# chechaohp/gan-ode

Measured on AMD Instinct MI355X. Metric: generated videos/sec (16-frame clips), higher is better.
Workload: dtype f32

## Files before the change

### gan-ode_amd/_lib.py

```python
from __future__ import annotations

import ctypes as C
import os
import sys

_HERE = os.path.dirname(os.path.abspath(__file__))
LIB_PATH = os.path.join(_HERE, "lib", "libgode.so")

i32, i64, f32, ptr = C.c_int32, C.c_int64, C.c_float, C.c_void_p
cint, u32, u64 = C.c_int, C.c_uint32, C.c_uint64

ACT_NONE, ACT_RELU, ACT_LRELU, ACT_TANH_OUT = 0, 1, 2, 3
ACT_TANH, ACT_SIGMOID = 4, 5
ACT_LRELU01 = 6
EPI_RAW, EPI_TANH = 0, 1
FPROP, DGRAD = 0, 1
PACK_BORDER = 0x100
OP_IGEMM, OP_WGRAD, OP_BN_FINALIZE, OP_BN_BWD, OP_ODE_FWD, OP_ODE_BWD, OP_BCE, OP_ADAM, OP_PACK = range(1, 10)
OP_ODERNN_FWD, OP_ODERNN_BWD, OP_BN_APPLY, OP_COL2IM = 10, 11, 12, 13
OP_SDE_FWD, OP_SDE_BWD = 14, 15
OP_CDE_FWD, OP_CDE_BWD = 16, 17
OP_WGAN = 18
OP_GRU_FWD, OP_GRU_BWD = 19, 20
OP_DNOISE = 21
OP_CATEG, OP_CE = 22, 23
OP_CHSTATS, OP_CBN_EMBED, OP_CBN_EMBED_BWD, OP_CBN_APPLY, OP_CBN_BWD, OP_GRES_OUT, OP_GRES_OUT_BWD, OP_SN_FWD, OP_SN_BWD = range(24, 33)
OP_FC_ACT, OP_FC_ACT_BWD, OP_BCE_PROB = 33, 34, 35
OP_BCE_T = 36
OP_RESIZE_U8, OP_CLIP_GATHER = 37, 38
RESIZE_MAX_TAPS = 32
REC_ADAM_NOISE = -1
ODE_NPARAM = 2672
ODERNN_NPARAM = 2176
SDE_NPARAM = 3216
CDE_NPARAM = 7536
CDE_MAX_N = 4096
GRU_NPARAM = 1632
SN_BWD_BLOCKS = 64
ODE_METHODS = {"rk4": 0, "dopri5": 1, "euler": 2, "midpoint": 3}
ODE_RHS = {"mlp": 0, "tanh": 1}
ODE_RHS_TANH_NPARAM = 2400


def ode_method_code(name):
# ... 27 lines not shown
    KIND, FN = OP_IGEMM, "gode_igemm"


class WgradOp(_Op):
    _fields_ = [("g", ConvGeom), ("act", i32), ("xform_on_y", i32), ("splits", i32), ("accumulate", i32),
                ("x", ptr), ("y", ptr), ("scale", ptr), ("shift", ptr), ("work", ptr), ("dw", ptr),
                ("co_perm", ptr), ("co_canon", i64), ("xs", i64 * 5)]
    KIND, FN = OP_WGRAD, "gode_wgrad"


class BnFinalizeOp(_Op):
    _fields_ = [("stats", ptr), ("rows", i32), ("ncols", i32), ("C", i32), ("count", i64), ("gamma", ptr),
                ("beta", ptr), ("running_mean", ptr), ("running_var", ptr), ("num_batches_tracked", ptr),
                ("mean", ptr), ("invstd", ptr), ("scale", ptr), ("shift", ptr), ("momentum", f32), ("eps", f32),
                ("training", i32), ("pad_", i32), ("groups", i32), ("rows0", i32), ("nseg", i32), ("order", i32),
                ("count1", i64), ("seg", i32 * 24), ("stats1", ptr), ("rows1", i32), ("pad3_", i32)]
    KIND, FN = OP_BN_FINALIZE, "gode_bn_finalize"


class BnBwdOp(_Op):
    _fields_ = [("g", ptr), ("y", ptr), ("M", i64), ("C", i32), ("act", i32), ("gamma", ptr), ("mean", ptr),
                ("invstd", ptr), ("scale", ptr), ("shift", ptr), ("dgamma", ptr), ("dbeta", ptr), ("work", ptr),
                ("accumulate", i32), ("eval_mode", i32), ("gin", ptr), ("groups", i32), ("pad2_", i32), ("M0", i64),
                ("r1_s", ptr), ("r1_w", ptr), ("r1_H", i32), ("r1_W", i32), ("r1_h", i32), ("r1_wd", i32), ("r1_off", i32),
                ("pad3_", i32)]
    KIND, FN = OP_BN_BWD, "gode_bn_bwd"


class OdeParams(C.Structure):
    _fields_ = [(n, ptr) for n in "Wa ba Wb bb W1 b1 W2 b2".split()]


# ... 271 lines not shown
    "gode_scale": ([ptr, ptr, i64, f32, cint, ptr], cint),
    "gode_adam_multi": ([ptr, i32, i64, f32, f32, f32, f32, f32, f32, i32, ptr], cint),
    "gode_adam_multi_dev": ([ptr, i32, i64, f32, f32, f32, f32, f32, ptr, ptr], cint),
    "gode_adam_noise_multi": ([ptr, i32, i64, f32, f32, f32, f32, f32, f32, i32, u64, u32, u32, f32, ptr], cint),
    "gode_adam_noise_multi_dev": ([ptr, i32, i64, f32, f32, f32, f32, f32, ptr, u64, u32, f32, ptr], cint),
    "gode_param_noise": ([ptr, i64, u64, u32, u32, i64, f32, i32, ptr], cint),
    "gode_dnoise_normals": ([ptr, i64, u64, u32, u32, u32, i64, i32, ptr], cint),
    "gode_ode_step_chunks": ([ptr, i64], i64),
    "gode_ode_step": ([ptr, i32, i64, i32, f32, f32, f32, f32, f32, ptr, ptr], cint),
    "gode_axpy_multi": ([ptr, i32, i64, f32, ptr, ptr, f32, ptr, ptr, ptr], cint),
    "gode_run": ([ptr, ptr, i32, ptr], cint),
    "gode_lanes_create": ([ptr], cint),
    "gode_lanes_destroy": ([ptr], cint),
    "gode_lanes_stream": ([ptr], ptr),
    "gode_run_lanes": ([ptr, ptr, ptr, i32, i32, i32, i32, ptr], cint),
    "gode_version": (None, cint),
    "gode_sizeof": ([cint], cint),
}

EXPORTS = [st.FN for st in _OPS] + list(_PROTOS)

_lib = None


def lib():
    global _lib
    if _lib is not None:
        return _lib
    if not os.path.exists(LIB_PATH):
        raise RuntimeError(f"{LIB_PATH} is missing: build it with `python __graft_entry__.py` "
# ... 63 lines not shown

class Lanes:

    _free = {}

    def __init__(self, device_index):
        self.device_index = device_index
        pool = Lanes._free.setdefault(device_index, [])
        if pool:
            self.handle = pool.pop()
        else:
            self.handle = ptr()
            check(lib().gode_lanes_create(C.byref(self.handle)), "gode_lanes_create")
        self.stream_ptr = lib().gode_lanes_stream(self.handle)

    def __del__(self):
        h, self.handle = getattr(self, "handle", None), None
        if h and not sys.is_finalizing():
            Lanes._free.setdefault(self.device_index, []).append(h)


class LanesProgram(Program):

    def __init__(self, ops, n_front, release_after):
        super().__init__(ops)
        self.n_front, self.release_after = int(n_front), int(release_after)

    def run_lanes(self, lanes, mode, stream):
        global LAUNCHES
        LAUNCHES += 1
        check(lib().gode_run_lanes(lanes.handle, self.kinds, self.ptrs, self.n, self.n_front, self.release_after, mode,
                                   stream), "gode_run_lanes")


def run_one(op, stream):
    global LAUNCHES
    LAUNCHES += 1
    if op.KIND == OP_PACK:
        launch = lambda: check(lib().gode_pack_weights(C.byref(op.g), op.dir, op.w, op.wpack, op.co_perm, op.co_canon,
                                                       stream), "gode_pack_weights")
        return _traced(op, stream, launch) if TRACE is not None else launch()
    if TRACE is not None:
        return _traced(op, stream, lambda: _run_one(op, stream))
    _run_one(op, stream)


def _run_one(op, stream):
# ... 2 lines not shown
```

### gan-ode_amd/csrc/api.hip

```cpp
#include "common.h"

extern "C" int gode_version(void) { return GODE_VERSION; }

extern "C" int gode_sizeof(int kind) {
  switch (kind) {
    case 0: return (int)sizeof(gode_conv_geom);
    case -1: return (int)sizeof(gode_adam_noise_tensor);
    case GODE_OP_PACK: return (int)sizeof(gode_pack_op);
#define GODE_SIZEOF_ROW_(name, value, op_t, fn) case GODE_OP_##name: return (int)sizeof(op_t);
    GODE_OPS(GODE_SIZEOF_ROW_)
#undef GODE_SIZEOF_ROW_
  }
  return GODE_E_KIND;
}

extern "C" int gode_pack_batch_(const gode_pack_op* const* ops, int n, void* stream);

static int run_range(const int32_t* kinds, const void* const* ops, int lo, int hi, void* stream) {
  for (int i = lo; i < hi; ++i) {
    int rc;
    switch (kinds[i]) {
#define GODE_RUN_ROW_(name, value, op_t, fn) case GODE_OP_##name: rc = fn((const op_t*)ops[i], stream); break;
      GODE_OPS(GODE_RUN_ROW_)
#undef GODE_RUN_ROW_
// ... 8 lines not shown
    }
    if (rc != 0) return rc > 0 ? rc : rc * 1000 - i;
  }
  return 0;
}

extern "C" int gode_run(const int32_t* kinds, const void* const* ops, int32_t n, void* stream) {
  if (n < 0 || (n > 0 && (!kinds || !ops))) return GODE_E_ARG;
  return run_range(kinds, ops, 0, n, stream);
}

struct gode_lanes {
  hipStream_t side;
  hipEvent_t ev_entry, ev_front, ev_release;
  bool released;
};

#define GODE_HIP_TRY(expr)                          \
  do {                                              \
    hipError_t e__ = (expr);                        \
    if (e__ != hipSuccess) return (int)e__;         \
  } while (0)

extern "C" int gode_lanes_destroy(gode_lanes* l) {
  if (!l) return GODE_E_ARG;
  int rc = 0;
  if (l->side) {
    hipError_t e = hipStreamSynchronize(l->side);
    if (e != hipSuccess) rc = (int)e;
  }
// ... 23 lines not shown
}

extern "C" void* gode_lanes_stream(gode_lanes* l) { return l ? (void*)l->side : nullptr; }

extern "C" int gode_run_lanes(gode_lanes* l, const int32_t* kinds, const void* const* ops, int32_t n, int32_t n_front,
                              int32_t release_after, int32_t mode, void* stream) {
  if (!l || n < 0 || (n > 0 && (!kinds || !ops)) || n_front < 0 || n_front > n || release_after < n_front ||
      release_after >= n || (mode != GODE_LANES_ORDERED && mode != GODE_LANES_OVERLAP))
    return GODE_E_ARG;
  hipStream_t main = (hipStream_t)stream;
  hipStreamCaptureStatus cap = hipStreamCaptureStatusNone;
  if (hipStreamIsCapturing(main, &cap) != hipSuccess) {
    (void)hipGetLastError();
    cap = hipStreamCaptureStatusActive;
  }
  if (cap != hipStreamCaptureStatusNone) {
    l->released = false;
    return run_range(kinds, ops, 0, n, stream);
  }
  const bool overlap = mode == GODE_LANES_OVERLAP && l->released;
  l->released = false;
  if (overlap) {
    GODE_HIP_TRY(hipStreamWaitEvent(l->side, l->ev_release, 0));
  } else {
    GODE_HIP_TRY(hipEventRecord(l->ev_entry, main));
    GODE_HIP_TRY(hipStreamWaitEvent(l->side, l->ev_entry, 0));
  }
  int rc = run_range(kinds, ops, 0, n_front, (void*)l->side);
  if (rc != 0) return rc;
  GODE_HIP_TRY(hipEventRecord(l->ev_front, l->side));
  GODE_HIP_TRY(hipStreamWaitEvent(main, l->ev_front, 0));
  rc = run_range(kinds, ops, n_front, release_after + 1, stream);
  if (rc != 0) return rc;
  GODE_HIP_TRY(hipEventRecord(l->ev_release, main));
  l->released = true;
  rc = run_range(kinds, ops, release_after + 1, n, stream);
  if (rc != 0) l->released = false;
  return rc;
}
```

### gan-ode_amd/csrc/elementwise.hip

```cpp
#include "common.h"
#include "philox.h"
#include "col2im_plan.h"

__global__ void __launch_bounds__(256) bn_finalize_kernel(const gode_bn_finalize_op a) {
  const int c = blockIdx.x, tid = threadIdx.x;
  __shared__ double red[2][256];
  if (a.training) {
    const int reps = a.ncols / a.C;
    const int ngroups = a.groups == 2 ? 2 : 1;
    for (int gi = 0; gi < ngroups; ++gi) {
      const int grp = ngroups == 2 ? (a.order ? 1 - gi : gi) : 0;
      double s1 = 0.0, s2 = 0.0;
      const int nseg = (ngroups == 2 && !a.stats1) ? (a.nseg > 0 ? a.nseg : 1) : 1;
      for (int sg = 0; sg < nseg; ++sg) {
        int r_lo, r_hi;
        if (ngroups == 1 || a.stats1) { r_lo = 0; r_hi = (grp == 1 && a.stats1) ? a.rows1 : a.rows; }
        else if (a.nseg > 0) { r_lo = grp == 0 ? a.seg[3 * sg] : a.seg[3 * sg + 1]; r_hi = grp == 0 ? a.seg[3 * sg + 1] : a.seg[3 * sg + 2]; }
        else { r_lo = grp == 0 ? 0 : a.rows0; r_hi = grp == 0 ? a.rows0 : a.rows; }
        const float* st = (grp == 1 && a.stats1) ? a.stats1 : a.stats;
        const int stride = (grp == 1 && a.stats1) ? a.rows1 : a.rows;
        const int nr = r_hi - r_lo;
        const int64_t items = (int64_t)nr * reps;
        for (int64_t i = tid; i < items; i += 256) {
          const int rep = (int)(i / nr); const int r = r_lo + (int)(i - (int64_t)rep * nr);
// ... 8 lines not shown
      for (int s = 128; s > 0; s >>= 1) {
        if (tid < s) { red[0][tid] += red[0][tid + s]; red[1][tid] += red[1][tid + s]; }
        __syncthreads();
      }
      if (tid == 0) {
        const double n = (double)((grp == 1 && a.count1 > 0) ? a.count1 : a.count);
        const double mean = red[0][0] / n;
        double var = red[1][0] / n - mean * mean;
        if (var < 0.0) var = 0.0;
        const float invstd = (float)(1.0 / sqrt(var + (double)a.eps));
        const float g = a.gamma ? a.gamma[c] : 1.f, b = a.beta ? a.beta[c] : 0.f;
        const float sc = g * invstd;
        const int o = grp * a.C + c;
        a.mean[o] = (float)mean; a.invstd[o] = invstd;
        a.scale[o] = sc; a.shift[o] = b - (float)mean * sc;
        if (a.running_mean) {
          const double unbiased = n > 1.0 ? var * n / (n - 1.0) : var;
          a.running_mean[c] = (1.f - a.momentum) * a.running_mean[c] + a.momentum * (float)mean;
          a.running_var[c] = (1.f - a.momentum) * a.running_var[c] + a.momentum * (float)unbiased;
        }
        if (c == 0 && a.num_batches_tracked) *a.num_batches_tracked += 1;
      }
    }
  } else if (tid == 0) {
    const float invstd = 1.f / sqrtf(a.running_var[c] + a.eps);
    const float g = a.gamma ? a.gamma[c] : 1.f, b = a.beta ? a.beta[c] : 0.f;
    const float sc = g * invstd;
    const int ngroups = a.groups == 2 ? 2 : 1;
    for (int grp = 0; grp < ngroups; ++grp) {
      const int o = grp * a.C + c;
      if (a.mean) a.mean[o] = a.running_mean[c];
      if (a.invstd) a.invstd[o] = invstd;
      a.scale[o] = sc; a.shift[o] = b - a.running_mean[c] * sc;
    }
  }
}

extern "C" int gode_bn_finalize(const gode_bn_finalize_op* op, void* stream) {
  if (!op || op->C <= 0 || !op->scale || !op->shift) return GODE_E_ARG;
  if (op->training) {
    if (!op->stats || !op->mean || !op->invstd || op->ncols % op->C != 0 || op->count <= 0) return GODE_E_ARG;
    if (op->stats1 && (op->groups != 2 || op->rows1 <= 0 || op->rows <= 0)) return GODE_E_ARG;
    if (op->groups == 2 && !op->stats1 && op->nseg == 0 && (op->rows0 <= 0 || op->rows0 >= op->rows)) return GODE_E_ARG;
    if (op->groups == 2 && (op->nseg < 0 || op->nseg > 8)) return GODE_E_ARG;
    for (int i = 0; op->groups == 2 && i < op->nseg; ++i)
      if (!(0 <= op->seg[3 * i] && op->seg[3 * i] <= op->seg[3 * i + 1] && op->seg[3 * i + 1] <= op->seg[3 * i + 2] && op->seg[3 * i + 2] <= op->rows)) return GODE_E_ARG;
  } else if (!op->running_mean || !op->running_var) return GODE_E_ARG;
  hipLaunchKernelGGL(bn_finalize_kernel, dim3(op->C), dim3(256), 0, (hipStream_t)stream, *op);
  GODE_LAUNCH_CHECK();
  return 0;
}

__global__ void __launch_bounds__(256) bn_apply_kernel(const gode_bn_apply_op a) {
  const int64_t n4 = a.M * a.C / 4;
  const float neg = gode_act_neg_slope(a.act);
  for (int64_t i = (int64_t)blockIdx.x * 256 + threadIdx.x; i < n4; i += (int64_t)gridDim.x * 256) {
    const int c = (int)((i * 4) % a.C) + ((a.M0 > 0 && i * 4 >= a.M0 * a.C) ? a.C : 0);
    f32x4 v = *reinterpret_cast<const f32x4*>(a.y + i * 4);
    f32x4 sc = {1.f, 1.f, 1.f, 1.f}, sh = {0.f, 0.f, 0.f, 0.f};
    if (a.scale) { sc = *reinterpret_cast<const f32x4*>(a.scale + c); sh = *reinterpret_cast<const f32x4*>(a.shift + c); }
#pragma unroll
    for (int e = 0; e < 4; ++e) { const float t = v[e] * sc[e] + sh[e]; v[e] = fmaxf(t, t * neg); }
    *reinterpret_cast<f32x4*>(a.out + i * 4) = v;
// ... 619 lines not shown
```

### gan-ode_amd/engine.py

```python
from __future__ import annotations

import ctypes as C
import os
from dataclasses import dataclass
from typing import List, Optional, Sequence

import numpy as np
import torch

from . import _lib as L

BORDER_TAKE_DEAD_TAPS = 0.06
BORDER_TAKE_TILES_PER_SLOT = 2.0


def border_value(g) -> int:
    lib = L.lib()
    if lib.gode_igemm_dead_taps(C.byref(L.IgemmOp(g=g, dir=L.DGRAD, tile=0))) < BORDER_TAKE_DEAD_TAPS:
        return 1
    info = (C.c_int32 * 4)()
    L.check(lib.gode_igemm_launch_info(C.byref(L.IgemmOp(g=g, dir=L.DGRAD, tile=0, border=2)), info))
    return 2 if info[0] and info[2] >= BORDER_TAKE_TILES_PER_SLOT * info[3] else 1


# ... 62 lines not shown
    return (i - back) % n


def lane_gate(prev_lanes, prev_copy_pending, before_prev_copy_pending):
    return bool(prev_copy_pending) if prev_lanes else bool(before_prev_copy_pending)


def lane_mode(*, enabled, trace, recording, categorical, grad, keep, fixed_grid_ode, splittable, prev_lanes, launches_between,
              repacked, versions_same, same_stream, gpu_behind=True):
    if (not enabled or trace or recording or categorical or grad or keep or not fixed_grid_ode or not splittable
            or not gpu_behind):
        return LANE_SINGLE
    if prev_lanes and launches_between == 0 and not repacked and versions_same and same_stream:
        return LANE_OVERLAP
    return LANE_ORDERED


@dataclass
class LayerSpec:
    geom: L.ConvGeom
    fwd_dir: int
    act: int
    has_bn: bool
    epilogue: int = L.EPI_RAW
    co_perm: Optional[torch.Tensor] = None
    noise: bool = False

    def out_dims(self):
        g = self.geom
        if self.fwd_dir == L.FPROP:
# ... 134 lines not shown
            L.Program(stale).run(st)
        return bool(stale)

    def front_split(self, prog, pre_ops):
        first = prog.ops[0] if prog.ops else None
        if (self.split or self.groups != 1 or self.noisy or self.x_in is None or len(prog.ops) < 2
                or not isinstance(first, L.IgemmOp) or first.out != dptr(self.y[0])):
            return None
        lib = L.lib()
        ops = list(pre_ops) + list(prog.ops)
        n_front = len(pre_ops) + 1
        written = front_writes(ops[:n_front], uses_work=lambda op: lib.gode_igemm_work_size(C.byref(op)) > 0)
        extents = {t.data_ptr(): t.numel() * t.element_size()
                   for t in (self.x_in, self.y[0], self.stats[0], self._ig_work) if t is not None}
        return ops, n_front, release_after(ops, n_front, written, extents)

    @staticmethod
    def _ncols(s: LayerSpec):
        g = s.geom
        if s.fwd_dir == L.FPROP:
            return g.Co
        fullk = (g.Do == 1 and g.Ho == 1 and g.Wo == 1 and g.pd == 0 and g.ph == 0 and g.pw == 0 and
                 g.Di == g.kd and g.Hi == g.kh and g.Wi == g.kw and g.kd * g.kh * g.kw > 1)
        return g.kd * g.kh * g.kw * g.Ci if fullk else g.Ci

    def _materialize(self, l):
        if l + 1 >= len(self.specs):
            return False
        if self.specs[l + 1].noise:
            return True
# ... 266 lines not shown
            if k is not None:
                x, xs = inputs[k]
                op.x = x.data_ptr()
                for i in range(5):
                    op.xs[i] = int(xs[i])

    def forward(self, training: bool, x: Optional[torch.Tensor] = None, x_strides=None, pre_ops_program=None,
                x2: Optional[torch.Tensor] = None, x2_strides=None, noise=None):
        prog, out, _ = self.begin_forward(training, x, x_strides, x2, x2_strides, noise)
        st = stream_ptr()
        if pre_ops_program is not None:
            pre_ops_program.run(st)
        prog.run(st)
        return self.end_forward(out, training)

    def begin_forward(self, training: bool, x=None, x_strides=None, x2=None, x2_strides=None, noise=None):
        self._refresh()
        if training not in self._fwd:
            self._fwd[training] = self._build_fwd(training)
        prog, patch = self._fwd[training]
        if self.noisy:
            if noise is None:
                raise RuntimeError("this plan applies instance noise: forward() needs its noise arguments")
            self._patch_noise(patch, noise, [(x, x_strides), (x2, x2_strides)])
        out = torch.empty(self.out_dims, dtype=torch.float32, device=self.device)
        patch["last"].out = out.data_ptr()
        if "last2" in patch:
            patch["last2"][0].out = out.data_ptr() + patch["last2"][1]
        if self.x_in is None and self.x0n is None:
            first = patch["first"]
            first.src = x.data_ptr()
            for i in range(5):
                first.gs[i] = int(x_strides[i])
        if self.x_in is None:
            self._x_user, self._x_strides = x.detach(), tuple(int(v) for v in x_strides)
            if self.groups == 2:
                if self.x0n is None:
                    second = patch["first2"]
                    second.src = x2.data_ptr()
                    for i in range(5):
# ... 267 lines not shown
```

### gan-ode_amd/modules.py

```python
from __future__ import annotations

import contextlib
import ctypes as C
import math
import os
from typing import Optional

import numpy as np
import torch
import torch.nn as nn

from . import _lib as L
from .engine import (LANE_ORDERED, LANE_OVERLAP, LANE_SINGLE, ConvStack, LayerParams, LayerSpec, conv_out, dptr, lane_gate,
                     lane_mode, make_geom, ring_back, stream_ptr)

Z_COLS = 96
Z_CATEG0 = 66
MAX_CATEG = Z_COLS - Z_CATEG0
ODE_METHODS = L.ODE_METHODS
_SAMPLE_LANES_ENV = os.environ.get("GODE_SAMPLE_LANES", "1") != "0"


def ode_method_code(name):
    return L.ode_method_code(name)


def _require_gpu(t: torch.Tensor, what: str):
    if not t.is_cuda:
        raise RuntimeError(f"{what}: this implementation runs only on an MI355X through libgode.so; move the module "
                           "to the GPU with .cuda() (there is no CPU or PyTorch fallback)")


class _Pool:

    MAX_PLANS = 6
# ... 170 lines not shown
_ODE_GRAD_OFFS = [(0, 1024, (64, 16)), (1024, 64, (64,)), (1088, 1024, (16, 64)), (2112, 16, (16,)),
                  (2128, 256, (16, 16)), (2384, 16, (16,)), (2400, 256, (16, 16)), (2656, 16, (16,))]
_PRENET_NPARAM = 2128


class _GenPlan:

    zcols = 68
    rows_in_traj = True
    rhs = property(lambda self: L.ode_rhs_code("tanh" if _is_one_layer(self.gen.ode_fn) else "mlp"))
    nparam = property(lambda self: L.ODE_RHS_TANH_NPARAM if self.rhs else L.ODE_NPARAM)
    grad_offs = property(lambda self: _ODE_GRAD_OFFS[:6] if self.rhs else _ODE_GRAD_OFFS)
    grads_from_first_present = False
    multi, multi_always = ("ode", L.OdeFwdOp, L.OdeBwdOp), False

    def __init__(self, gen: "VideoGenerator", n_traj: int, T: int, select: bool, zbuf=None, x=None):
        dev = gen.main[0].weight.device
        self.gen, self.n, self.T, self.select, self.device = gen, n_traj, T, select, dev
        self.rows = n_traj if select else n_traj * T
        f32 = dict(dtype=torch.float32, device=dev)
        self.ncat = int(getattr(gen, "dim_z_category", 0)) if x is None else 0
        self.labels = None
        self.x, self.content, self.sel, self.cls = x, None, None, None
        self._ring = []
        if x is None:
            xs = self._x_shape(n_traj, T)
            sx, sc, ss, sk = _input_slices(int(np.prod(xs)), n_traj)
            nin = sk.stop if self.ncat else sk.start
            self._in = torch.zeros(nin, **f32)
            self.x, self.content = self._in[sx].view(xs), self._in[sc].view(n_traj, 50)
            self.sel = self._in[ss].view(torch.int32) if select else None
# ... 2 lines not shown
        self._ring_i = 0
        self.stack = None
        if x is not None:
            self._zbuf, self._zcols = torch.empty(n_traj * T, self.zcols, **f32), self.zcols
        elif zbuf is not None:
            self._zbuf, self._zcols = zbuf, Z_COLS
        else:
            self.stack = ConvStack(gen._decoder_specs(self.rows), gen._decoder_params(), dev, owns_input=True,
                                   pack_cache=gen._pool.pack_cache, two_lane_backward=True)
            self._zbuf, self._zcols = self.stack.x_in, Z_COLS
        self._alloc()
        self._ode_ptrs = None
        self.busy = False
        self._lanes = self._side = self._lane_prog = self._lane_prev = None
        self.lane_calls = {LANE_OVERLAP: 0, LANE_ORDERED: 0, LANE_SINGLE: 0}
        self._lanes_ok = type(self) is _GenPlan and self.stack is not None and not self.ncat and _SAMPLE_LANES_ENV
        self.lanes_made_late = False
        if self._lanes_ok and gen.sample_lanes:
            self._make_lanes()

    @staticmethod
    def _x_shape(n_traj, T):
        return (n_traj, 16)

    def _alloc(self):
        f32 = dict(dtype=torch.float32, device=self.device)
        self.traj = torch.empty(self.n, self.T, 16, **f32)
        tt = torch.linspace(0, 1, self.T).float()
        self.dt = (tt[1:] - tt[:-1]).to(self.device) if self.T > 1 else torch.zeros(1, **f32)
        self.ode_work = torch.empty(L.lib().gode_ode_bwd_work_size(self.n), **f32)

    def _params(self):
        g = self.gen
# ... 88 lines not shown
        if feed is not None and feed.recording:
            nfl = self._in.numel()
            pin, dev = feed.noise_region(self.gen, self.select, self.n, self.T, nfl)
            _pack_inputs(pin, x_host, content_host, sel_host, cls_host)
            self._in.copy_(dev)
        else:
            slot = self._ring[self._ring_i]
            self._ring_i = (self._ring_i + 1) % len(self._ring)
            if slot["ev"] is not None:
                slot["ev"].synchronize()
            _pack_inputs(slot["buf"], x_host, content_host, sel_host, cls_host)
            self._in.copy_(slot["buf"], non_blocking=True)
            if slot["ev"] is None:
                slot["ev"] = torch.cuda.Event()
            slot["ev"].record()

    def forward(self, x_host, content_host, sel_host, training, keep, cls_host=None, no_grad=False):
        if x_host is None:
            torch.cuda.current_stream().wait_event(self._latent_ev)
            out = self.stack.forward(training)
            self._lane_prev = None
        elif self._lanes_possible(keep, no_grad):
            out = self._forward_lanes(x_host, content_host, sel_host, training)
        else:
            self.stage_inputs(x_host, content_host, sel_host, cls_host)
            out = self.stack.forward(training, pre_ops_program=self.fwd_prog)
            self._lane_prev = None
            self.lane_calls[LANE_SINGLE] += 1
        self.busy = keep
        return out

    def _lanes_possible(self, keep, no_grad):
        gen = self.gen
        if (not no_grad or keep or not gen.sample_lanes or gen._one_stream or not self._lanes_ok or L.TRACE is not None
                or gen.ode_method == "dopri5"):
            return False
        if gen.sample_lanes != "always" and not lane_gate(self._lane_prev is not None, self._copy_pending(1),
                                                          self._copy_pending(2)):
            return False
        feed = getattr(gen, "_feed", None)
        if (feed is not None and feed.recording) or torch.cuda.is_current_stream_capturing():
            return False
        if self._lanes is None:
            self._make_lanes()
            self.lanes_made_late = True
        return True

    def _copy_pending(self, back):
        ev = self._ring[ring_back(self._ring_i, len(self._ring), back)]["ev"]
        return ev is not None and not ev.query()

    def _make_lanes(self):
        with torch.cuda.device(self.device):
            self._lanes = L.Lanes(torch.cuda.current_device())
        self._side = torch.cuda.ExternalStream(self._lanes.stream_ptr, device=self.device)

    def _front_versions(self):
        ts = [t for t in self._params() if t is not None] + [self.stack.params[0].weight]
        return tuple((t._version, getattr(t, "_gode_ver", 0), t.data_ptr()) for t in ts)

    def _forward_lanes(self, x_host, content_host, sel_host, training):
        self._programs()
        prev, self._lane_prev = self._lane_prev, None
        between = L.LAUNCHES - prev["mark"] if prev is not None else -1
        prog, out, repacked = self.stack.begin_forward(training)
        st = stream_ptr()
        cache = self._lane_prog
        if cache is None or cache[0] is not prog or cache[1] is not self.fwd_prog:
            split = self.stack.front_split(prog, self.fwd_prog.ops)
# ... 19 lines not shown
        return self.stack.end_forward(out, training)

    def _stage_on_side(self, ordered, x_host, content_host, sel_host):
        slot = self._ring[self._ring_i]
        self._ring_i = (self._ring_i + 1) % len(self._ring)
        if slot["ev"] is not None:
            slot["ev"].synchronize()
        _pack_inputs(slot["buf"], x_host, content_host, sel_host)
        if ordered:
            self._side.wait_stream(torch.cuda.current_stream())
        with torch.cuda.stream(self._side):
            self._in.copy_(slot["buf"], non_blocking=True)
            if slot["ev"] is None:
                slot["ev"] = torch.cuda.Event()
            slot["ev"].record()

    def _decoder_pass_done(self):
        cb = getattr(self.gen, "_on_decoder_grads", None)
        if cb is not None:
            self.gen._decoder_passes_left -= 1
            if self.gen._decoder_passes_left == 0:
                cb()

    def backward(self, gout, arena=None):
        if arena is not None:
            into = _grads_into(arena, self.gen._decoder_params())
            _, _, gz = self.stack.backward(gout, need_input_grad=True, into=into)
            self._decoder_pass_done()
            self.latent_backward(gz.data_ptr(), arena, gz)
            self.busy = False
# ... 277 lines not shown
        if not isinstance(self.linear, nn.Identity):
            ode += [self.linear[0].weight, self.linear[0].bias, self.linear[2].weight, self.linear[2].bias]
        ode += _ode_fn_tensors(self.ode_fn)
        return self._decoder_list(), ode

    def _apply(self, fn, *a, **k):
        r = super()._apply(fn, *a, **k)
        if hasattr(self, "_pool"):
            self._pool.clear()
            self.__dict__.pop("_labels", None)
            self.__dict__.pop("_latent_plans", None)
            self.__dict__.pop("_prefetched", None)
        return r

    def lane_stats(self):
        out = {LANE_OVERLAP: 0, LANE_ORDERED: 0, LANE_SINGLE: 0, "lanes_objects": 0, "lanes_objects_made_late": 0}
        for plans in self._pool.plans.values():
            for p in plans:
                for k, v in getattr(p, "lane_calls", {}).items():
                    out[k] += v
                out["lanes_objects"] += getattr(p, "_lanes", None) is not None
                out["lanes_objects_made_late"] += bool(getattr(p, "lanes_made_late", False))
        return out

    @contextlib.contextmanager
    def one_stream(self):
        self._one_stream += 1
        try:
            yield
        finally:
            self._one_stream -= 1

    def invalidate_packs(self):
        for k in [k for k in self._pool.pack_cache if k[0] == "ver"]:
            del self._pool.pack_cache[k]
        for plans in self._pool.plans.values():
            for p in plans:
                if getattr(p, "_lane_prev", None) is not None:
                    p._lane_prev = None

    def _zero_labels(self, n, device):
        key = (n, device)
        t = self.__dict__.setdefault("_labels", {}).get(key)
        if t is None:
            t = self._labels[key] = torch.zeros(n, dtype=torch.float64, device=device)
        return t

    _gode_direct_grads = True

    def _arena_tail(self):
        return self._param_list()[1]

    def _draw(self, num_samples, video_len):
        content = np.random.normal(0, 1, (num_samples, self.dim_z_content)).astype(np.float32)
# ... 1025 lines not shown
```

### include/gode.h

```cpp
#ifndef GODE_H
#define GODE_H
#include <stdint.h>
#ifdef __cplusplus
extern "C" {
#endif

#define GODE_VERSION 105

enum { GODE_OK = 0, GODE_E_ARG = -1, GODE_E_SHAPE = -2, GODE_E_KIND = -3 };
enum { GODE_ACT_NONE = 0, GODE_ACT_RELU = 1, GODE_ACT_LRELU = 2,
       GODE_ACT_TANH_OUT = 3 ,
       GODE_ACT_TANH = 4, GODE_ACT_SIGMOID = 5 ,
       GODE_ACT_LRELU01 = 6  };
enum { GODE_EPI_RAW = 0, GODE_EPI_TANH = 1 };
enum { GODE_FPROP = 0, GODE_DGRAD = 1 };
enum { GODE_PACK_BORDER = 0x100 };

typedef struct gode_conv_geom {
  int32_t N, Ci, Co;
  int32_t Di, Hi, Wi;
  int32_t Do, Ho, Wo;
  int32_t kd, kh, kw;
  int32_t sd, sh, sw;
  int32_t pd, ph, pw;
// ... 40 lines not shown
  int64_t xs[5];
} gode_wgrad_op;
int gode_wgrad(const gode_wgrad_op* op, void* stream);
int64_t gode_wgrad_work_size(const gode_wgrad_op* op);
int gode_wgrad_auto_splits(const gode_conv_geom* g);

typedef struct gode_bn_finalize_op {
  const float* stats; int32_t rows, ncols, C; int64_t count;
  const float* gamma; const float* beta;
  float* running_mean; float* running_var; int64_t* num_batches_tracked;
  float* mean; float* invstd; float* scale; float* shift;
  float momentum, eps; int32_t training, pad_;
  int32_t groups, rows0;
  int32_t nseg, order; int64_t count1; int32_t seg[24];
  const float* stats1; int32_t rows1, pad3_;
} gode_bn_finalize_op;
int gode_bn_finalize(const gode_bn_finalize_op* op, void* stream);

typedef struct gode_bn_apply_op {
  const float* y; float* out; const float* scale; const float* shift; int64_t M; int32_t C, act;
  int64_t M0;
} gode_bn_apply_op;
int gode_bn_apply(const gode_bn_apply_op* op, void* stream);

typedef struct gode_col2im_op {
  const float* cols; float* out;
  int32_t N, Hi, Wi, Ho, Wo, C, kh, kw, sh, sw, ph, pw;
  int32_t epilogue, pad_;
  int32_t Di, Do, kd, sd, pd, pad2_;
} gode_col2im_op;
int gode_col2im(const gode_col2im_op* op, void* stream);
int gode_col2im_launch_kind(const gode_col2im_op* op, int32_t* kind);
// ... 323 lines not shown
  X(CE,            23, gode_ce_op,            gode_ce_logits)     \
  X(CHSTATS,       24, gode_chstats_op,       gode_chstats)       \
  X(CBN_EMBED,     25, gode_cbn_embed_op,     gode_cbn_embed)     \
  X(CBN_EMBED_BWD, 26, gode_cbn_embed_bwd_op, gode_cbn_embed_bwd) \
  X(CBN_APPLY,     27, gode_cbn_apply_op,     gode_cbn_apply)     \
  X(CBN_BWD,       28, gode_cbn_bwd_op,       gode_cbn_bwd)       \
  X(GRES_OUT,      29, gode_gres_out_op,      gode_gres_out)      \
  X(GRES_OUT_BWD,  30, gode_gres_out_bwd_op,  gode_gres_out_bwd)  \
  X(SN_FWD,        31, gode_sn_op,            gode_sn_fwd)        \
  X(SN_BWD,        32, gode_sn_bwd_op,        gode_sn_bwd)        \
  X(FC_ACT,        33, gode_fc_act_op,        gode_fc_act)        \
  X(FC_ACT_BWD,    34, gode_fc_act_bwd_op,    gode_fc_act_bwd)    \
  X(BCE_PROB,      35, gode_bce_prob_op,      gode_bce_prob)      \
  X(BCE_T,         36, gode_bce_t_op,         gode_bce_logits_t)  \
  X(RESIZE_U8,     37, gode_resize_u8_op,     gode_resize_u8)     \
  X(CLIP_GATHER,   38, gode_clip_gather_op,   gode_clip_gather)
#define GODE_ENUM_ROW_(name, value, op_t, fn) GODE_OP_##name = value,
enum { GODE_OPS(GODE_ENUM_ROW_) GODE_OP_PACK = 9 };
#undef GODE_ENUM_ROW_
typedef struct gode_pack_op {
  gode_conv_geom g; int32_t dir , co_canon; const float* w; float* wpack; const int32_t* co_perm;
} gode_pack_op;
int gode_run(const int32_t* kinds, const void* const* ops, int32_t n, void* stream);

typedef struct gode_lanes gode_lanes;
enum { GODE_LANES_ORDERED = 0, GODE_LANES_OVERLAP = 1 };
int gode_lanes_create(gode_lanes** out);
int gode_lanes_destroy(gode_lanes* lanes);
void* gode_lanes_stream(gode_lanes* lanes);
int gode_run_lanes(gode_lanes* lanes, const int32_t* kinds, const void* const* ops, int32_t n, int32_t n_front,
                   int32_t release_after, int32_t mode, void* stream);

int gode_version(void);
int gode_sizeof(int kind);

#ifdef __cplusplus
}
#endif
#endif
```

Before: 39280.

## Double-buffer generator sampling across two plans with deferred BN running-stat update

Adds a paired execution mode in which consecutive training-mode sampling calls alternate between two plan copies on separate side streams. When overlap is allowed, each call's front waits on the peer's entry event rather than its own, so two forward passes can run concurrently. BN finalize now writes the batch variance to a scratch buffer, and a single trailing BN_RUNNING kernel on the main stream applies the running-mean/var updates in order, keeping the shared running statistics race-free. This costs a second set of buffers and lanes, one extra launch per call, and more complex ordering logic.

```diff
diff --git a/gan-ode_amd/_lib.py b/gan-ode_amd/_lib.py
--- a/gan-ode_amd/_lib.py
+++ b/gan-ode_amd/_lib.py
@@ -28,6 +28,8 @@
 OP_FC_ACT, OP_FC_ACT_BWD, OP_BCE_PROB = 33, 34, 35
 OP_BCE_T = 36
 OP_RESIZE_U8, OP_CLIP_GATHER = 37, 38
+OP_BN_RUNNING = 39
+BN_RUNNING_MAX = 8
 RESIZE_MAX_TAPS = 32
 REC_ADAM_NOISE = -1
 ODE_NPARAM = 2672
@@ -85,8 +87,18 @@
                 ("beta", ptr), ("running_mean", ptr), ("running_var", ptr), ("num_batches_tracked", ptr),
                 ("mean", ptr), ("invstd", ptr), ("scale", ptr), ("shift", ptr), ("momentum", f32), ("eps", f32),
                 ("training", i32), ("pad_", i32), ("groups", i32), ("rows0", i32), ("nseg", i32), ("order", i32),
-                ("count1", i64), ("seg", i32 * 24), ("stats1", ptr), ("rows1", i32), ("pad3_", i32)]
+                ("count1", i64), ("seg", i32 * 24), ("stats1", ptr), ("rows1", i32), ("pad3_", i32), ("batch_var", ptr)]
     KIND, FN = OP_BN_FINALIZE, "gode_bn_finalize"
+
+
+class BnRunningLayer(C.Structure):
+    _fields_ = [("mean", ptr), ("var", ptr), ("running_mean", ptr), ("running_var", ptr), ("num_batches_tracked", ptr),
+                ("C", i32), ("pad_", i32)]
+
+
+class BnRunningOp(_Op):
+    _fields_ = [("layer", BnRunningLayer * BN_RUNNING_MAX), ("n", i32), ("momentum", f32)]
+    KIND, FN = OP_BN_RUNNING, "gode_bn_running"
 
 
 class BnBwdOp(_Op):
@@ -388,6 +400,7 @@
     "gode_lanes_destroy": ([ptr], cint),
     "gode_lanes_stream": ([ptr], ptr),
     "gode_run_lanes": ([ptr, ptr, ptr, i32, i32, i32, i32, ptr], cint),
+    "gode_run_pair": ([ptr, ptr, ptr, ptr, i32, i32, i32, ptr], cint),
     "gode_version": (None, cint),
     "gode_sizeof": ([cint], cint),
 }
@@ -481,6 +494,15 @@
             check(lib().gode_lanes_create(C.byref(self.handle)), "gode_lanes_create")
         self.stream_ptr = lib().gode_lanes_stream(self.handle)
 
+    _shared = {}
+
+    @classmethod
+    def shared(cls, device_index, second):
+        key = (device_index, bool(second))
+        if key not in cls._shared:
+            cls._shared[key] = cls(device_index)
+        return cls._shared[key]
+
     def __del__(self):
         h, self.handle = getattr(self, "handle", None), None
         if h and not sys.is_finalizing():
@@ -498,6 +520,19 @@
         LAUNCHES += 1
         check(lib().gode_run_lanes(lanes.handle, self.kinds, self.ptrs, self.n, self.n_front, self.release_after, mode,
                                    stream), "gode_run_lanes")
+
+
+class PairProgram(Program):
+
+    def __init__(self, ops, n_tail=1):
+        super().__init__(ops)
+        self.n_tail = int(n_tail)
+
+    def run_pair(self, lanes, peer, mode, stream):
+        global LAUNCHES
+        LAUNCHES += 1
+        check(lib().gode_run_pair(lanes.handle, None if peer is None else peer.handle, self.kinds, self.ptrs, self.n,
+                                  self.n_tail, mode, stream), "gode_run_pair")
 
 
 def run_one(op, stream):
diff --git a/gan-ode_amd/csrc/api.hip b/gan-ode_amd/csrc/api.hip
--- a/gan-ode_amd/csrc/api.hip
+++ b/gan-ode_amd/csrc/api.hip
@@ -46,6 +46,7 @@
   hipStream_t side;
   hipEvent_t ev_entry, ev_front, ev_release;
   bool released;
+  bool entered;
 };
 
 #define GODE_HIP_TRY(expr)                          \
@@ -99,6 +100,7 @@
     (void)hipGetLastError();
     cap = hipStreamCaptureStatusActive;
   }
+  l->entered = false;
   if (cap != hipStreamCaptureStatusNone) {
     l->released = false;
     return run_range(kinds, ops, 0, n, stream);
@@ -123,3 +125,30 @@
   if (rc != 0) l->released = false;
   return rc;
 }
+
+extern "C" int gode_run_pair(gode_lanes* l, gode_lanes* peer, const int32_t* kinds, const void* const* ops, int32_t n,
+                             int32_t n_tail, int32_t mode, void* stream) {
+  if (!l || peer == l || n < 2 || !kinds || !ops || n_tail < 1 || n_tail >= n ||
+      (mode != GODE_LANES_ORDERED && mode != GODE_LANES_OVERLAP))
+    return GODE_E_ARG;
+  hipStream_t main = (hipStream_t)stream;
+  hipStreamCaptureStatus cap = hipStreamCaptureStatusNone;
+  if (hipStreamIsCapturing(main, &cap) != hipSuccess) {
+    (void)hipGetLastError();
+    cap = hipStreamCaptureStatusActive;
+  }
+  l->released = false;
+  l->entered = false;
+  if (cap != hipStreamCaptureStatusNone) return run_range(kinds, ops, 0, n, stream);
+  const bool overlap = mode == GODE_LANES_OVERLAP && peer && peer->entered;
+  GODE_HIP_TRY(hipEventRecord(l->ev_entry, main));
+  GODE_HIP_TRY(hipStreamWaitEvent(l->side, overlap ? peer->ev_entry : l->ev_entry, 0));
+  int rc = run_range(kinds, ops, 0, n - n_tail, (void*)l->side);
+  GODE_HIP_TRY(hipEventRecord(l->ev_front, l->side));
+  GODE_HIP_TRY(hipStreamWaitEvent(main, l->ev_front, 0));
+  if (rc != 0) return rc;
+  rc = run_range(kinds, ops, n - n_tail, n, stream);
+  if (rc != 0) return rc;
+  l->entered = true;
+  return 0;
+}
diff --git a/gan-ode_amd/csrc/elementwise.hip b/gan-ode_amd/csrc/elementwise.hip
--- a/gan-ode_amd/csrc/elementwise.hip
+++ b/gan-ode_amd/csrc/elementwise.hip
@@ -1,6 +1,18 @@
 #include "common.h"
 #include "philox.h"
 #include "col2im_plan.h"
+
+__device__ __forceinline__ float bn_running_mean_update(float run, float momentum, float batch_mean) {
+#pragma clang fp contract(off)
+  const float keep = (1.f - momentum) * run;
+  const float add = momentum * batch_mean;
+  return add + keep;
+}
+__device__ __forceinline__ float bn_running_var_update(float run, float momentum, float unbiased) {
+#pragma clang fp contract(off)
+  const float keep = (1.f - momentum) * run;
+  return __builtin_fmaf(momentum, unbiased, keep);
+}
 
 __global__ void __launch_bounds__(256) bn_finalize_kernel(const gode_bn_finalize_op a) {
   const int c = blockIdx.x, tid = threadIdx.x;
@@ -46,12 +58,16 @@
         const int o = grp * a.C + c;
         a.mean[o] = (float)mean; a.invstd[o] = invstd;
         a.scale[o] = sc; a.shift[o] = b - (float)mean * sc;
-        if (a.running_mean) {
-          const double unbiased = n > 1.0 ? var * n / (n - 1.0) : var;
-          a.running_mean[c] = (1.f - a.momentum) * a.running_mean[c] + a.momentum * (float)mean;
-          a.running_var[c] = (1.f - a.momentum) * a.running_var[c] + a.momentum * (float)unbiased;
+        if (a.batch_var) {
+          a.batch_var[c] = (float)(n > 1.0 ? var * n / (n - 1.0) : var);
+        } else {
+          if (a.running_mean) {
+            const double unbiased = n > 1.0 ? var * n / (n - 1.0) : var;
+            a.running_mean[c] = bn_running_mean_update(a.running_mean[c], a.momentum, (float)mean);
+            a.running_var[c] = bn_running_var_update(a.running_var[c], a.momentum, (float)unbiased);
+          }
+          if (c == 0 && a.num_batches_tracked) *a.num_batches_tracked += 1;
         }
-        if (c == 0 && a.num_batches_tracked) *a.num_batches_tracked += 1;
       }
     }
   } else if (tid == 0) {
@@ -78,7 +94,32 @@
     for (int i = 0; op->groups == 2 && i < op->nseg; ++i)
       if (!(0 <= op->seg[3 * i] && op->seg[3 * i] <= op->seg[3 * i + 1] && op->seg[3 * i + 1] <= op->seg[3 * i + 2] && op->seg[3 * i + 2] <= op->rows)) return GODE_E_ARG;
   } else if (!op->running_mean || !op->running_var) return GODE_E_ARG;
+  if (op->batch_var && (!op->training || op->groups == 2 || op->nseg != 0 || op->stats1)) return GODE_E_ARG;
   hipLaunchKernelGGL(bn_finalize_kernel, dim3(op->C), dim3(256), 0, (hipStream_t)stream, *op);
+  GODE_LAUNCH_CHECK();
+  return 0;
+}
+
+__global__ void __launch_bounds__(256) bn_running_kernel(const gode_bn_running_op a) {
+  for (int l = 0; l < a.n; ++l) {
+    const gode_bn_running_layer& y = a.layer[l];
+    if (y.running_mean)
+      for (int c = threadIdx.x; c < y.C; c += 256) {
+        y.running_mean[c] = bn_running_mean_update(y.running_mean[c], a.momentum, y.mean[c]);
+        y.running_var[c] = bn_running_var_update(y.running_var[c], a.momentum, y.var[c]);
+      }
+    if (threadIdx.x == 0 && y.num_batches_tracked) *y.num_batches_tracked += 1;
+    __syncthreads();
+  }
+}
+
+extern "C" int gode_bn_running(const gode_bn_running_op* op, void* stream) {
+  if (!op || op->n <= 0 || op->n > GODE_BN_RUNNING_MAX) return GODE_E_ARG;
+  for (int l = 0; l < op->n; ++l) {
+    const gode_bn_running_layer& y = op->layer[l];
+    if (y.C <= 0 || (y.running_mean && (!y.running_var || !y.mean || !y.var))) return GODE_E_ARG;
+  }
+  hipLaunchKernelGGL(bn_running_kernel, dim3(1), dim3(256), 0, (hipStream_t)stream, *op);
   GODE_LAUNCH_CHECK();
   return 0;
 }
diff --git a/gan-ode_amd/engine.py b/gan-ode_amd/engine.py
--- a/gan-ode_amd/engine.py
+++ b/gan-ode_amd/engine.py
@@ -100,6 +100,25 @@
     if prev_lanes and launches_between == 0 and not repacked and versions_same and same_stream:
         return LANE_OVERLAP
     return LANE_ORDERED
+
+
+def pair_turn(prev_turn):
+    return 0 if prev_turn is None else 1 - prev_turn
+
+
+def pair_wait(turn, overlap):
+    return 1 - turn if overlap else turn
+
+
+def pair_schedule(calls):
+    out, entry, prev = [], {}, None
+    for m, (fresh, may_overlap) in enumerate(calls):
+        turn = pair_turn(None if fresh else prev)
+        overlap = bool(may_overlap) and not fresh and (1 - turn) in entry
+        entry[turn] = m
+        out.append((turn, entry[pair_wait(turn, overlap)]))
+        prev = turn
+    return out
 
 
 @dataclass
@@ -264,6 +283,31 @@
         extents = {t.data_ptr(): t.numel() * t.element_size()
                    for t in (self.x_in, self.y[0], self.stats[0], self._ig_work) if t is not None}
         return ops, n_front, release_after(ops, n_front, written, extents)
+
+    def pair_program(self, prog, pre_ops):
+        if self.split or self.groups != 1 or self.noisy or self.x_in is None or len(prog.ops) < 2:
+            return None
+        fins = [op for op in prog.ops if isinstance(op, L.BnFinalizeOp)]
+        if not fins or len(fins) > L.BN_RUNNING_MAX or any(not f.training or f.groups == 2 or f.nseg or f.stats1 for f in fins):
+            return None
+        if getattr(self, "_bvar", None) is None:
+            self._bvar = {}
+        run = L.BnRunningOp(n=len(fins), momentum=self.momentum)
+        ops, k = list(pre_ops), -1
+        for op in prog.ops:
+            if isinstance(op, L.BnFinalizeOp):
+                k += 1
+                slot = self._bvar.get(k)
+                if slot is None or slot.numel() != op.C:
+                    slot = self._bvar[k] = torch.empty(op.C, dtype=torch.float32, device=self.device)
+                d = L.BnFinalizeOp.from_buffer_copy(op)
+                d.batch_var = slot.data_ptr()
+                y = run.layer[k]
+                y.mean, y.var, y.C = op.mean, slot.data_ptr(), op.C
+                y.running_mean, y.running_var, y.num_batches_tracked = op.running_mean, op.running_var, op.num_batches_tracked
+                op = d
+            ops.append(op)
+        return ops + [run]
 
     @staticmethod
     def _ncols(s: LayerSpec):
@@ -560,7 +604,7 @@
         prog.run(st)
         return self.end_forward(out, training)
 
-    def begin_forward(self, training: bool, x=None, x_strides=None, x2=None, x2_strides=None, noise=None):
+    def begin_forward(self, training: bool, x=None, x_strides=None, x2=None, x2_strides=None, noise=None, out_stream=None):
         self._refresh()
         if training not in self._fwd:
             self._fwd[training] = self._build_fwd(training)
@@ -569,7 +613,13 @@
             if noise is None:
                 raise RuntimeError("this plan applies instance noise: forward() needs its noise arguments")
             self._patch_noise(patch, noise, [(x, x_strides), (x2, x2_strides)])
-        out = torch.empty(self.out_dims, dtype=torch.float32, device=self.device)
+        if out_stream is None:
+            out = torch.empty(self.out_dims, dtype=torch.float32, device=self.device)
+        else:
+            cur = torch.cuda.current_stream()
+            with torch.cuda.stream(out_stream):
+                out = torch.empty(self.out_dims, dtype=torch.float32, device=self.device)
+            out.record_stream(cur)
         patch["last"].out = out.data_ptr()
         if "last2" in patch:
             patch["last2"][0].out = out.data_ptr() + patch["last2"][1]
diff --git a/gan-ode_amd/modules.py b/gan-ode_amd/modules.py
--- a/gan-ode_amd/modules.py
+++ b/gan-ode_amd/modules.py
@@ -12,13 +12,14 @@
 
 from . import _lib as L
 from .engine import (LANE_ORDERED, LANE_OVERLAP, LANE_SINGLE, ConvStack, LayerParams, LayerSpec, conv_out, dptr, lane_gate,
-                     lane_mode, make_geom, ring_back, stream_ptr)
+                     lane_mode, make_geom, pair_turn, stream_ptr)
 
 Z_COLS = 96
 Z_CATEG0 = 66
 MAX_CATEG = Z_COLS - Z_CATEG0
 ODE_METHODS = L.ODE_METHODS
 _SAMPLE_LANES_ENV = os.environ.get("GODE_SAMPLE_LANES", "1") != "0"
+_PAIR_DEFAULT = True
 
 
 def ode_method_code(name):
@@ -219,7 +220,7 @@
     grads_from_first_present = False
     multi, multi_always = ("ode", L.OdeFwdOp, L.OdeBwdOp), False
 
-    def __init__(self, gen: "VideoGenerator", n_traj: int, T: int, select: bool, zbuf=None, x=None):
+    def __init__(self, gen: "VideoGenerator", n_traj: int, T: int, select: bool, zbuf=None, x=None, lanes=None):
         dev = gen.main[0].weight.device
         self.gen, self.n, self.T, self.select, self.device = gen, n_traj, T, select, dev
         self.rows = n_traj if select else n_traj * T
@@ -252,9 +253,17 @@
         self.busy = False
         self._lanes = self._side = self._lane_prog = self._lane_prev = None
         self.lane_calls = {LANE_OVERLAP: 0, LANE_ORDERED: 0, LANE_SINGLE: 0}
+        self._peer = self._pair_prog = self._pair_prev = None
+        self._pair_refused = False
+        self._owner = self
+        self.pair_calls = {LANE_OVERLAP: 0, LANE_ORDERED: 0}
+        self._copies = []
         self._lanes_ok = type(self) is _GenPlan and self.stack is not None and not self.ncat and _SAMPLE_LANES_ENV
         self.lanes_made_late = False
-        if self._lanes_ok and gen.sample_lanes:
+        self._peer_lanes = None
+        if lanes is not None:
+            self._make_lanes(lanes)
+        elif self._lanes_ok and gen.sample_lanes:
             self._make_lanes()
 
     @staticmethod
@@ -373,18 +382,29 @@
             if slot["ev"] is None:
                 slot["ev"] = torch.cuda.Event()
             slot["ev"].record()
+            self._note_copy(slot["ev"])
+
+    def _note_copy(self, ev):
+        own = self._owner
+        own._copies = own._copies[-1:] + [ev]
 
     def forward(self, x_host, content_host, sel_host, training, keep, cls_host=None, no_grad=False):
         if x_host is None:
             torch.cuda.current_stream().wait_event(self._latent_ev)
             out = self.stack.forward(training)
-            self._lane_prev = None
+            self._lane_prev = self._pair_prev = None
         elif self._lanes_possible(keep, no_grad):
-            out = self._forward_lanes(x_host, content_host, sel_host, training)
+            knob = self.gen.sample_lanes
+            if (knob == "pair" or (_PAIR_DEFAULT and knob != "always")) and self._pair_possible(training):
+                self._lane_prev = None
+                out = self._forward_pair(x_host, content_host, sel_host, training)
+            else:
+                self._pair_prev = None
+                out = self._forward_lanes(x_host, content_host, sel_host, training)
         else:
             self.stage_inputs(x_host, content_host, sel_host, cls_host)
             out = self.stack.forward(training, pre_ops_program=self.fwd_prog)
-            self._lane_prev = None
+            self._lane_prev = self._pair_prev = None
             self.lane_calls[LANE_SINGLE] += 1
         self.busy = keep
         return out
@@ -394,8 +414,8 @@
         if (not no_grad or keep or not gen.sample_lanes or gen._one_stream or not self._lanes_ok or L.TRACE is not None
                 or gen.ode_method == "dopri5"):
             return False
-        if gen.sample_lanes != "always" and not lane_gate(self._lane_prev is not None, self._copy_pending(1),
-                                                          self._copy_pending(2)):
+        if gen.sample_lanes not in ("always", "pair") and not lane_gate(
+                self._lane_prev is not None or self._pair_prev is not None, self._copy_pending(1), self._copy_pending(2)):
             return False
         feed = getattr(gen, "_feed", None)
         if (feed is not None and feed.recording) or torch.cuda.is_current_stream_capturing():
@@ -406,12 +426,15 @@
         return True
 
     def _copy_pending(self, back):
-        ev = self._ring[ring_back(self._ring_i, len(self._ring), back)]["ev"]
+        ev = self._copies[-back] if len(self._copies) >= back else None
         return ev is not None and not ev.query()
 
-    def _make_lanes(self):
+    def _make_lanes(self, lanes=None):
         with torch.cuda.device(self.device):
-            self._lanes = L.Lanes(torch.cuda.current_device())
+            self._lanes = lanes if lanes is not None else L.Lanes.shared(torch.cuda.current_device(), False)
+            knob = self.gen.sample_lanes
+            if lanes is None and (knob == "pair" or (_PAIR_DEFAULT and knob != "always")):
+                self._peer_lanes = L.Lanes.shared(torch.cuda.current_device(), True)
         self._side = torch.cuda.ExternalStream(self._lanes.stream_ptr, device=self.device)
 
     def _front_versions(self):
@@ -461,6 +484,51 @@
             if slot["ev"] is None:
                 slot["ev"] = torch.cuda.Event()
             slot["ev"].record()
+        self._note_copy(slot["ev"])
+
+    def _pair_possible(self, training):
+        return training and not self._pair_refused and self.stack._G2 is False and not self.stack.noisy
+
+    def _pair_versions(self):
+        ts = [t for t in self._params() if t is not None]
+        for p in self.stack.params:
+            ts += [t for t in (p.weight, p.gamma, p.beta) if t is not None]
+        return tuple((t._version, getattr(t, "_gode_ver", 0), t.data_ptr()) for t in ts)
+
+    def _forward_pair(self, x_host, content_host, sel_host, training):
+        prev, self._pair_prev = self._pair_prev, None
+        turn = pair_turn(None if prev is None else prev["turn"])
+        if turn == 1 and self._peer is None:
+            if self._peer_lanes is None:
+                with torch.cuda.device(self.device):
+                    self._peer_lanes = L.Lanes.shared(torch.cuda.current_device(), True)
+            peer = self._peer = type(self)(self.gen, self.n, self.T, self.select, lanes=self._peer_lanes)
+            peer._owner = self
+        plan = self._peer if turn else self
+        plan._programs()
+        between = L.LAUNCHES - prev["mark"] if prev is not None else -1
+        prog, out, repacked = plan.stack.begin_forward(training, out_stream=plan._side)
+        st = stream_ptr()
+        cache = plan._pair_prog
+        if cache is None or cache[0] is not prog or cache[1] is not plan.fwd_prog:
+            ops = plan.stack.pair_program(prog, plan.fwd_prog.ops)
+            if ops is None:
+                self._pair_refused = True
+                return self._forward_lanes(x_host, content_host, sel_host, training)
+            cache = plan._pair_prog = (prog, plan.fwd_prog, L.PairProgram(ops, 1))
+            prev = None
+        versions = self._pair_versions()
+        mode = lane_mode(enabled=True, trace=False, recording=False, categorical=False, grad=False, keep=False,
+                         fixed_grid_ode=True, splittable=True, prev_lanes=prev is not None, launches_between=between,
+                         repacked=repacked, versions_same=prev is not None and prev["versions"] == versions,
+                         same_stream=prev is not None and prev["stream"] == st, gpu_behind=True)
+        self.pair_calls[mode] += 1
+        plan._stage_on_side(mode == LANE_ORDERED, x_host, content_host, sel_host)
+        other = self if turn else self._peer
+        cache[2].run_pair(plan._lanes, None if other is None else other._lanes,
+                          L.LANES_OVERLAP if mode == LANE_OVERLAP else L.LANES_ORDERED, st)
+        self._pair_prev = dict(mark=L.LAUNCHES, versions=versions, stream=st, turn=turn)
+        return plan.stack.end_forward(out, training)
 
     def _decoder_pass_done(self):
         cb = getattr(self.gen, "_on_decoder_grads", None)
@@ -768,11 +836,15 @@
         return r
 
     def lane_stats(self):
-        out = {LANE_OVERLAP: 0, LANE_ORDERED: 0, LANE_SINGLE: 0, "lanes_objects": 0, "lanes_objects_made_late": 0}
+        out = {LANE_OVERLAP: 0, LANE_ORDERED: 0, LANE_SINGLE: 0, "lanes_objects": 0, "lanes_objects_made_late": 0,
+               "pair_overlap": 0, "pair_ordered": 0, "pair_plans": 0}
         for plans in self._pool.plans.values():
             for p in plans:
                 for k, v in getattr(p, "lane_calls", {}).items():
                     out[k] += v
+                for k, v in getattr(p, "pair_calls", {}).items():
+                    out["pair_" + k] += v
+                out["pair_plans"] += getattr(p, "_peer", None) is not None
                 out["lanes_objects"] += getattr(p, "_lanes", None) is not None
                 out["lanes_objects_made_late"] += bool(getattr(p, "lanes_made_late", False))
         return out
@@ -792,6 +864,8 @@
             for p in plans:
                 if getattr(p, "_lane_prev", None) is not None:
                     p._lane_prev = None
+                if getattr(p, "_pair_prev", None) is not None:
+                    p._pair_prev = None
 
     def _zero_labels(self, n, device):
         key = (n, device)
diff --git a/include/gode.h b/include/gode.h
--- a/include/gode.h
+++ b/include/gode.h
@@ -78,8 +78,20 @@
   int32_t groups, rows0;
   int32_t nseg, order; int64_t count1; int32_t seg[24];
   const float* stats1; int32_t rows1, pad3_;
+  float* batch_var;
 } gode_bn_finalize_op;
 int gode_bn_finalize(const gode_bn_finalize_op* op, void* stream);
+
+#define GODE_BN_RUNNING_MAX 8
+typedef struct gode_bn_running_layer {
+  const float* mean; const float* var; float* running_mean; float* running_var; int64_t* num_batches_tracked;
+  int32_t C, pad_;
+} gode_bn_running_layer;
+typedef struct gode_bn_running_op {
+  gode_bn_running_layer layer[8];
+  int32_t n; float momentum;
+} gode_bn_running_op;
+int gode_bn_running(const gode_bn_running_op* op, void* stream);
 
 typedef struct gode_bn_apply_op {
   const float* y; float* out; const float* scale; const float* shift; int64_t M; int32_t C, act;
@@ -433,7 +445,8 @@
   X(BCE_PROB,      35, gode_bce_prob_op,      gode_bce_prob)      \
   X(BCE_T,         36, gode_bce_t_op,         gode_bce_logits_t)  \
   X(RESIZE_U8,     37, gode_resize_u8_op,     gode_resize_u8)     \
-  X(CLIP_GATHER,   38, gode_clip_gather_op,   gode_clip_gather)
+  X(CLIP_GATHER,   38, gode_clip_gather_op,   gode_clip_gather)   \
+  X(BN_RUNNING,    39, gode_bn_running_op,    gode_bn_running)
 #define GODE_ENUM_ROW_(name, value, op_t, fn) GODE_OP_##name = value,
 enum { GODE_OPS(GODE_ENUM_ROW_) GODE_OP_PACK = 9 };
 #undef GODE_ENUM_ROW_
@@ -449,6 +462,8 @@
 void* gode_lanes_stream(gode_lanes* lanes);
 int gode_run_lanes(gode_lanes* lanes, const int32_t* kinds, const void* const* ops, int32_t n, int32_t n_front,
                    int32_t release_after, int32_t mode, void* stream);
+int gode_run_pair(gode_lanes* lanes, gode_lanes* peer, const int32_t* kinds, const void* const* ops, int32_t n,
+                  int32_t n_tail, int32_t mode, void* stream);
 
 int gode_version(void);
 int gode_sizeof(int kind);
```

Result: faster. 42850, median of 6 (+9.1%).
